# Kiteretsu77/This_and_That_VDM

Hardware: AMD Instinct MI355X
Metric: denoise-steps/sec (14-frame 256x448 VGL, 25 steps) (higher is better)
Workload: dtype bf16; 1 GPU; VGL denoise step: GestureNet ControlNet + spatio-temporal UNet + per-frame CFG + Euler, latent 14x4x32x56, CFG batch 2, 78 context tokens, heads (5,10,20,20); mode=vgl, requests_per_gpu=1, parallelism=1 independent request(s), one per GPU; RCCL weight broadcast at start-up only, hipgraph=True, finite_output=True, spatial_self_attention=bf16, weights_identical_on_all_ranks=True

## Files before the change

### this_and_that_vdm_amd/csrc/gemm.hip

```cpp
#include <stdlib.h>
#include "gemm_kernel.h"

namespace ttg {
void launch_bf16(GemmP& p, int cfg, hipStream_t st);
void launch_f16(GemmP& p, int cfg, hipStream_t st);
void launch_f32(GemmP& p, int cfg, hipStream_t st);
void launch_sq320_bf16(const GemmP& p, hipStream_t st);
void launch_sq320_f16(const GemmP& p, hipStream_t st);
void launch_pp_bf16(GemmP& p, hipStream_t st);
void launch_pp_f16(GemmP& p, hipStream_t st);
void launch_w320(GemmP& p, hipStream_t st, int bm, bool bf16);
}
using namespace ttg;

namespace {
inline int gemm_taps(int mode) { return mode == 1 || mode == 3 ? 9 : (mode == 2 ? 3 : 1); }

int env_int(const char* name, int dflt) { const char* e = getenv(name); return e ? atoi(e) : dflt; }
int big_tile_bits(int on) { return on == 0 ? 0 : (on == 2 ? 1 : (on == 3 ? 11 : (on == 4 ? 7 : 15))); }
struct Knobs {
  int forced_cfg = env_int("TT_GEMM_CFG", -1);
  int group_m = env_int("TT_GEMM_GROUP_M", 0);
  int forced_split = env_int("TT_GEMM_SPLITK", -1);
  int deep = env_int("TT_GEMM_DEEP", 1);
  int small64 = env_int("TT_GEMM_SMALL64", 2);
  int sq320 = env_int("TT_GEMM_SQ320", 2);
  int sq320_rowvec = env_int("TT_SQ320_ROWVEC", 1);
  int sq320_min_rows = env_int("TT_SQ320_MIN_ROWS", 131072);
  int pp = env_int("TT_GEMM_PP", 1);
  int pp_geglu_min_tiles = env_int("TT_PP_GEGLU_MIN_TILES", 400);
  int pp_geglu_min_fill = env_int("TT_PP_GEGLU_MIN_FILL", 75);
  int pp_min_tiles = env_int("TT_PP_MIN_TILES", 460);
  int pp_min_fill = env_int("TT_PP_MIN_FILL", 90);
  int pp_split_whole = env_int("TT_PP_SPLIT_WHOLE", 1);
  int w320 = big_tile_bits(env_int("TT_GEMM_W320", 1));
  int w320_force = env_int("TT_W320_FORCE", 0);
  int w320_min_fill = env_int("TT_W320_MIN_FILL", 60);
  int f32_split = env_int("TT_F32_SPLIT", 0) ? 1 : 0;
  int f32_split_min_tiles = env_int("TT_F32_SPLIT_MIN_TILES", 160);
  int f32_splitk = env_int("TT_F32_SPLITK", 1);
};
Knobs& knobs() { static Knobs k; return k; }

struct Plan { int cfg, splitk; };

Plan make_plan(int forced, int m, int n, long ktot, bool allow_split, bool wide_ok = true, bool mode0 = false, bool k128 = false) {
  Plan pl{0, 1};
  const int f = forced;
  const long b128 = (long)ceil_div(m, 128) * ceil_div(n, 128);
  const long b12864 = (long)ceil_div(m, 128) * ceil_div(n, 64);
  if (f >= 0 && f < kNumCfgs) pl.cfg = f;
  else if (n % 160 == 0 && n % 128 != 0 && n <= 960 && m >= 2048) pl.cfg = 7;
  else if (m >= 8192 && n >= 1024 && wide_ok) pl.cfg = 3;
  else if (m < 2048 && n >= 2560 && n % 160 == 0) pl.cfg = 7;
  else if (b128 >= 384) pl.cfg = 11;
  else if (b12864 >= 384) pl.cfg = 1;
  else pl.cfg = 2;
  const int fs = knobs().forced_split;
  if (fs >= 1) { pl.splitk = allow_split ? fs : 1; return pl; }
  const long kt = (ktot + 63) / 64;
  const int deep = knobs().deep;
  if (deep && f < 0 && b128 <= 256 && ktot > 0) {
    const int small64 = knobs().small64;
    if (small64 && (small64 != 2 || (m <= 64 && n >= 4096)) && mode0 && ktot <= 2048 && (long)ceil_div(m, 64) * ceil_div(n, 64) <= 512) { pl.cfg = 2; return pl; }
    pl.cfg = (deep == 2 && k128) ? 20 : 16;
    long s = allow_split ? 256 / b128 : 1;
    if (s > kt / 8) s = kt / 8;
    if (s > 16) s = 16;
    pl.splitk = s >= 2 ? (int)s : 1;
    return pl;
  }
  if (allow_split && f < 0 && b128 < 384 && kt >= 40) {
    long s = (512 + b128 - 1) / b128;
    if (s > kt / 8) s = kt / 8;
    if (s > 16) s = 16;
    if (s >= 2) { pl.cfg = 11; pl.splitk = (int)s; }
  }
  return pl;
}

int plan_f32(int m, int n, int min_tiles = 256) { return (long)ceil_div(m, 128) * ceil_div(n, 128) >= min_tiles ? 0 : 1; }

bool sq320_rowvec_ok(const TtGemmArgs* a) {
  if (!a->rowvec) return true;
  if (!knobs().sq320_rowvec || !a->residual) return false;
  if (a->rowvec_mod == 2 && a->rowvec_rows == 1) return true;
  return a->rowvec_mod == 0 && a->rowvec_rows >= 32 && a->rowvec_rows % 32 == 0 && (long)a->rowvec_rows * 2 >= a->m;
}
bool sq320_ok(const TtGemmArgs* a) {
  const int on = knobs().sq320;
  if (on == 2 && a->m < knobs().sq320_min_rows) return false;
  return on && a->dtype != TT_F32 && !a->ln_fold && !a->out_fp8 && knobs().forced_cfg < 0 && a->mode == 0 && a->k1 == 0 && a->k0 == SQ_K && a->n == SQ_N && a->m >= 4096 &&
         !a->geglu && sq320_rowvec_ok(a) && !a->out_f32 && !a->out_col_hw &&
         (!a->blend || (a->blend == a->residual && a->ld_blend == a->ld_res));
}
bool pp_ok(const TtGemmArgs* a) {
  const Knobs& k = knobs();
  if (!k.pp || k.forced_cfg >= 0 || a->dtype == TT_F32 || a->mode != 0 || a->k1 != 0 || a->ln_fold > 1 || a->out_fp8 || a->residual || a->blend ||
      a->rowvec || a->out_f32 || a->out_col_hw || (a->k0 & 63) || a->k0 < 128 || (a->n & 15) || (a->ldo & 7))
    return false;
  const long tiles = (long)ceil_div(a->m, 256) * ceil_div(a->n, 256);
  const long rounds = (tiles + 255) / 256;
  if (a->geglu) return tiles >= k.pp_geglu_min_tiles && tiles * 100 >= rounds * 256 * k.pp_geglu_min_fill;
  return tiles >= k.pp_min_tiles && tiles * 100 >= rounds * 256 * k.pp_min_fill;
}
bool w320_eligible(const TtGemmArgs* a) {
  if (!knobs().w320 || knobs().forced_cfg >= 0 || a->mode == 3 || a->dtype == TT_F32 || a->n % 320 || (a->k0 & 63) || (a->k1 & 63) || gemm_taps(a->mode) * (a->k0 + a->k1) < 128 || a->geglu ||
      a->out_fp8 || a->out_f32 || a->out_col_hw || a->ln_fold > 1 || (a->ln_fold && (a->mode != 0 || a->k1)))
    return false;
  if (a->mode == 1 && (a->stride != 1 || a->upsample || a->hin != a->hout || a->win != a->wout || a->win >= 32768 || a->hin >= 32768)) return false;
  if (a->rowvec && a->rowvec_rows < 32 && !(a->rowvec_rows == 1 && a->rowvec_mod == 2)) return false;
  if ((a->ldo & 3) || (a->residual && (a->ld_res & 3)) || (a->blend && (a->ld_blend & 3)) || (a->rowvec && (a->ld_rowvec & 3))) return false;
  if ((((size_t)a->out | (size_t)a->residual | (size_t)a->blend) & 7) || (((size_t)a->rowvec | (size_t)a->bias) & 15)) return false;
  return true;
}
int w320_route(const TtGemmArgs* a) {
  if (!w320_eligible(a)) return 0;
// ... 176 lines not shown
extern "C" int32_t tt_gemm_gn_fused(const TtGemmArgs* a) {
  if (!a || a->m <= 0 || a->n <= 0) return 0;
  return gn_fused_on(a, resolve(a));
}

extern "C" size_t tt_gemm_ws_bytes(const TtGemmArgs* a) {
  if (!a || a->m <= 0 || a->n <= 0) return 0;
  const Route r = wanted_route(a);
  if (r.kind == Kind::PP_TWO_PART) { TtGemmArgs head, tail; pp_split(a, r.head_rows, &head, &tail); return tt_gemm_ws_bytes(&tail); }
  return (r.kind == Kind::W320H_SPLIT || r.kind == Kind::TILED) && r.splitk > 1 ? slab_bytes(a, r.splitk) : 0;
}

namespace {
int fill_params(const TtGemmArgs* a, const Route& r, GemmP& p) {
  if (a->geglu && ((a->n & 15) || a->residual || a->blend || a->rowvec || a->out_f32 || a->out_col_hw))
    TT_FAIL(TT_EINVAL, "tt_gemm: geglu needs n %% 16 == 0 and no other epilogue terms");
  if (a->rowvec && a->rowvec_rows <= 0) TT_FAIL(TT_EINVAL, "tt_gemm: rowvec_rows");
  if (a->gn_out) {
    if (!a->gn_gamma || !a->gn_beta || (a->ld_gn & 3) || ((size_t)a->gn_out & 7)) TT_FAIL(TT_EINVAL, "tt_gemm: gn_out needs gn_gamma, gn_beta, ld_gn %% 4 == 0 and an 8-byte aligned pointer");
    if (!gn_fused_on(a, r)) TT_FAIL(TT_EUNSUPPORTED, "tt_gemm: gn_out on a problem without a split-K reduction pass (tt_gemm_gn_fused(args) == 0)");
  }
  if (a->stats_out && stats_rows_on(a, r) == 0)
    TT_FAIL(TT_EUNSUPPORTED, "tt_gemm: stats_out on a route without a statistics epilogue (tt_gemm_stats_rows(args) == 0)");
  if (a->rowvec_mod < 0 || (a->rowvec_mod > 0 && !a->rowvec)) TT_FAIL(TT_EINVAL, "tt_gemm: rowvec_mod %d (>= 0, needs rowvec)", a->rowvec_mod);
  if (a->ln_fold < 0 || a->ln_fold > 2) TT_FAIL(TT_EINVAL, "tt_gemm: ln_fold %d (0 none, 1 rows of A, 2 rows of W)", a->ln_fold);
  if (a->ln_fold && (a->mode != 0 || a->k1 != 0 || !(a->ln_eps > 0.f)))
    TT_FAIL(TT_EINVAL, "tt_gemm: ln_fold needs mode 0, one source spanning the whole LayerNorm row (k0 = C) and ln_eps > 0");
  if (a->ln_fold == 2 && a->geglu) TT_FAIL(TT_EINVAL, "tt_gemm: ln_fold 2 (columns) cannot be combined with geglu");
  if (a->out_fp8 && (a->dtype == TT_F32 || a->mode != 0 || a->geglu || a->residual || a->blend || a->rowvec || a->out_f32 || (a->ldo & 3)))
    TT_FAIL(TT_EINVAL, "tt_gemm: out_fp8 is for plain 16-bit linears (no geglu / residual / blend / rowvec / fp32 out), ldo %% 4 == 0");
  p.a0 = (const char*)a->a0; p.a1 = (const char*)a->a1; p.k0 = a->k0; p.k1 = a->k1;
  p.lda0 = a->lda0; p.lda1 = a->lda1; p.w = (const char*)a->w; p.ldw = a->ldw;
  p.m = a->m; p.n = a->n; p.mode = a->mode;
  p.nimg = a->nimg; p.hin = a->hin; p.win = a->win; p.hout = a->hout; p.wout = a->wout;
  p.stride = a->stride; p.upsample = a->upsample; p.frames = a->frames; p.hw = a->hw;
  p.bias = a->bias; p.acc_scale = a->acc_scale;
  p.rowvec = a->rowvec; p.rowvec_rows = a->rowvec_rows; p.ld_rowvec = a->ld_rowvec; p.rowvec_mod = a->rowvec ? a->rowvec_mod : 0;
  p.geglu = a->geglu; p.residual = (const char*)a->residual; p.ld_res = a->ld_res;
  p.blend = (const char*)a->blend; p.ld_blend = a->ld_blend; p.alpha = a->alpha;
  const int es = a->dtype == TT_F32 ? 4 : 2;
  p.out = (char*)a->out; p.ldo = a->ldo; p.out_f32 = a->dtype == TT_F32 ? 0 : a->out_f32;
  p.out_col_hw = a->out_col_hw; p.out_col_hwp = a->out_col_hwp;
  p.ln_fold = a->ln_fold; p.ln_eps = a->ln_eps; p.out_fp8 = a->out_fp8; p.stats = a->stats_out; p.stat_rows = a->gn_out ? a->stats_seg : (a->stats_out ? stats_rows_on(a, r) : 0);
  p.f32_split = a->dtype == TT_F32 ? knobs().f32_split : 0;
  p.presplit = a->presplit;
  if (a->presplit) {
    if ((a->presplit & ~3) || a->dtype != TT_F32 || !p.f32_split)
      TT_FAIL(TT_EINVAL, "tt_gemm: presplit operands need TT_F32 with tt_gemm_set_f32_split(1)");
    if (((a->presplit & 1) && a->ln_fold == 1) || ((a->presplit & 2) && a->ln_fold == 2))
      TT_FAIL(TT_EINVAL, "tt_gemm: the LayerNorm statistics cannot be taken from a pre-split operand");
    if ((a->presplit & 1) && a->mode != 0) TT_FAIL(TT_EINVAL, "tt_gemm: a pre-split A operand is a Linear operand (mode 0)");
  }
  p.gn_out = (char*)a->gn_out; p.ld_gn = a->ld_gn; p.gn_gamma = a->gn_gamma; p.gn_beta = a->gn_beta; p.gn_eps = a->gn_eps; p.gn_silu = a->gn_silu;
  if (p.mode == 1 || p.mode == 3) {
    if (p.nimg <= 0 || p.hin <= 0 || p.win <= 0 || p.hout <= 0 || p.wout <= 0 || p.stride < 1)
      TT_FAIL(TT_EINVAL, "tt_gemm: conv geometry");
    if ((long)p.nimg * p.hout * p.wout != p.m) TT_FAIL(TT_EINVAL, "tt_gemm: m != nimg*hout*wout");
  }
  if (p.mode == 2) {
    if (p.frames <= 0 || p.hw <= 0 || p.m % ((long)p.frames * p.hw)) TT_FAIL(TT_EINVAL, "tt_gemm: tconv geometry");
  }
  p.taps = gemm_taps(p.mode);
  {
    const long rows = p.mode == 1 || p.mode == 3 ? (long)p.nimg * p.hin * p.win : (long)p.m;
    const long a0b = ((rows - 1) * p.lda0 + p.k0) * es, a1b = p.k1 ? ((rows - 1) * p.lda1 + p.k1) * es : 16;
    const long wb = ((long)(p.n - 1) * p.ldw + (long)p.taps * (p.k0 + p.k1)) * es;
    if (a0b >= (1L << 31) || a1b >= (1L << 31) || wb >= (1L << 31))
      TT_FAIL(TT_EUNSUPPORTED, "tt_gemm: operand larger than 2 GiB (32-bit buffer offsets)");
    p.a0_bytes = (unsigned)a0b; p.a1_bytes = (unsigned)a1b; p.w_bytes = (unsigned)wb;
    const long n_out = p.geglu ? p.n / 2 : p.n;
    const long outb = ((long)(p.m - 1) * p.ldo + (p.out_col_hw > 0 ? p.ldo : n_out)) * (p.out_f32 ? 4 : (p.out_fp8 ? 1 : es));
    const long resb = p.residual ? ((long)(p.m - 1) * p.ld_res + p.n) * es : 0;
    const long blb = p.blend ? ((long)(p.m - 1) * p.ld_blend + p.n) * es : 0;
    long rv_last = p.rowvec ? (p.m - 1) / p.rowvec_rows : 0;
    if (p.rowvec_mod > 0 && rv_last > p.rowvec_mod - 1) rv_last = p.rowvec_mod - 1;
    const long rvb = p.rowvec ? (rv_last * p.ld_rowvec + p.n) * 4 : 0;
    if (outb >= (1L << 31) || resb >= (1L << 31) || blb >= (1L << 31) || rvb >= (1L << 31))
      TT_FAIL(TT_EUNSUPPORTED, "tt_gemm: epilogue operand larger than 2 GiB (32-bit buffer offsets)");
    p.out_bytes = (unsigned)outb; p.res_bytes = (unsigned)resb; p.blend_bytes = (unsigned)blb;
    p.bias_bytes = p.bias ? (unsigned)p.n * 4u : 0u; p.rowvec_bytes = (unsigned)rvb;
  }
  p.splitk = r.splitk; p.group_m = 1;
  p.group_m_override = r.kind == Kind::PP || r.kind == Kind::TILED ? knobs().group_m : 0;
  p.ws = r.splitk > 1 ? (float*)a->ws : nullptr;
  p.ws_bytes = r.splitk > 1 ? (unsigned)slab_bytes(a, r.splitk) : 0u;
  return TT_OK;
}
}

extern "C" int tt_gemm(const TtGemmArgs* a, tt_stream_t stream) {
  if (!a || !a->a0 || !a->w || !a->out) TT_FAIL(TT_EINVAL, "tt_gemm: null operand");
  if (a->m <= 0 || a->n <= 0 || a->k0 <= 0) TT_FAIL(TT_EINVAL, "tt_gemm: empty problem m=%d n=%d k0=%d", a->m, a->n, a->k0);
  if (a->dtype != TT_BF16 && a->dtype != TT_F16 && a->dtype != TT_F32) TT_FAIL(TT_EINVAL, "tt_gemm: bad dtype");
  if ((a->k0 & 7) || (a->k1 & 7) || (a->n & 3)) TT_FAIL(TT_EINVAL, "tt_gemm: k0/k1 must be multiples of 8 and n of 4");
  if ((a->lda0 & 7) || (a->k1 && (a->lda1 & 7)) || (a->ldw & 7)) TT_FAIL(TT_EINVAL, "tt_gemm: row strides must be multiples of 8 elements");
  if (a->k1 && !a->a1) TT_FAIL(TT_EINVAL, "tt_gemm: k1 > 0 without a1");
  if (a->mode < 0 || a->mode > 3) TT_FAIL(TT_EINVAL, "tt_gemm: bad mode %d", a->mode);
  if (a->mode == 3 && a->upsample) TT_FAIL(TT_EINVAL, "tt_gemm: mode 3 (bottom / right zero padding) has no fused upsample");
  const Route r = resolve(a);
  if (r.kind == Kind::PP_TWO_PART) {
    TtGemmArgs head, tail;
    pp_split(a, r.head_rows, &head, &tail);
    const int rc = tt_gemm(&head, stream);
    return rc != TT_OK ? rc : tt_gemm(&tail, stream);
  }
  GemmP p;
  if (const int rc = fill_params(a, r, p)) return rc;
  hipStream_t st = (hipStream_t)stream;
  const bool bf16 = a->dtype == TT_BF16;
  switch (r.kind) {
    case Kind::PP: if (bf16) launch_pp_bf16(p, st); else launch_pp_f16(p, st); break;
    case Kind::SQ320: if (bf16) launch_sq320_bf16(p, st); else launch_sq320_f16(p, st); break;
    case Kind::W320: launch_w320(p, st, 256, bf16); break;
    case Kind::W320H: case Kind::W320H_SPLIT: launch_w320(p, st, 128, bf16); break;
    case Kind::TILED:
      if (bf16) launch_bf16(p, r.cfg, st);
      else if (a->dtype == TT_F16) launch_f16(p, r.cfg, st);
      else launch_f32(p, r.cfg, st);
      break;
    default:
      TT_FAIL(TT_EUNSUPPORTED, "tt_gemm: forced tile configuration %d has no mode-3 variant (mode 3 is built for 1, 2, 11, 16)", r.cfg);
  }
  TT_CHECK_LAUNCH("tt_gemm");
  return TT_OK;
}
```

### this_and_that_vdm_amd/csrc/gemm_kernel.h

```cpp
#pragma once
#include <stdlib.h>
#include <type_traits>
#include "common.h"

namespace ttg {


struct FastDiv { unsigned mul, sh; };
static inline FastDiv make_fastdiv(long d_) {
  unsigned long long d = d_ < 1 ? 1 : (unsigned long long)d_;
  unsigned l = 0;
  while ((1ull << l) < d) ++l;
  FastDiv f;
  f.mul = (unsigned)(((1ull << (31 + l)) + d - 1) / d);
  f.sh = 31 + l;
  return f;
}
__device__ __forceinline__ int fdiv(int n, const FastDiv& f) { return (int)(((unsigned long long)(unsigned)n * f.mul) >> f.sh); }

struct GemmP {
  const char* a0; const char* a1;
  int k0, k1; long lda0, lda1;
  const char* w; long ldw;
  int m, n, mode;
  int nimg, hin, win, hout, wout, stride, upsample;
  int frames, hw;
  const float* bias; float acc_scale;
  const float* rowvec; int rowvec_rows; long ld_rowvec;
  int rowvec_mod;
  int geglu;
  const char* residual; long ld_res;
  const char* blend; long ld_blend; float alpha;
  char* out; long ldo; int out_f32;
  int out_col_hw, out_col_hwp;
  int nk0, nk1, taps, kt_total;
  int tiles_m, tiles_n;
  int group_m_override;
  int group_m;
  unsigned a0_bytes, a1_bytes, w_bytes;
  unsigned out_bytes, res_bytes, blend_bytes, bias_bytes, rowvec_bytes, ws_bytes;
  int splitk;
  float* ws;
  int ln_fold; float ln_eps;
  int out_fp8;
  float* stats;
  int stat_rows;
  char* gn_out; long ld_gn;
  const float* gn_gamma; const float* gn_beta; float gn_eps; int gn_silu;
  int f32_split;
  int presplit;
  FastDiv fd_splitk, fd_per_group, fd_group_m, fd_last_rows, fd_per_tap, fd_hwo, fd_wout, fd_hw, fd_frames, fd_rv_rows, fd_rv_mod;
};

__device__ __forceinline__ unsigned pack4_fp8(const float* v) {
  int w = 0;
  w = __builtin_amdgcn_cvt_pk_fp8_f32(__builtin_amdgcn_fmed3f(v[0], -448.f, 448.f), __builtin_amdgcn_fmed3f(v[1], -448.f, 448.f), w, false);
  w = __builtin_amdgcn_cvt_pk_fp8_f32(__builtin_amdgcn_fmed3f(v[2], -448.f, 448.f), __builtin_amdgcn_fmed3f(v[3], -448.f, 448.f), w, true);
  return (unsigned)w;
}
__device__ __forceinline__ void st32(__amdgpu_buffer_rsrc_t r, int off, unsigned a) {
  __builtin_amdgcn_raw_buffer_store_b32(a, r, off, 0, 0);
}

__device__ __forceinline__ void colstat_strip(const char* ebuf, int q_per_row, int lane, float* srow_sum, float* srow_sq, bool first) {
  if (lane < q_per_row * 4) {
    const int quad = lane >> 2, e4 = (lane & 3) * 4;
    float a = 0.f, b = 0.f;
#pragma unroll 8
    for (int r = 0; r < 32; ++r) {
      const float x = *(const float*)(ebuf + r * 256 + ((quad ^ (r & (q_per_row - 1))) << 4) + e4);
      a += x; b = fmaf(x, x, b);
    }
    if (!first) { a += srow_sum[lane]; b += srow_sq[lane]; }
    srow_sum[lane] = a; srow_sq[lane] = b;
  }
}

__device__ __forceinline__ void ln_stat_shifted(const raw_u32x4_t& f, float c, float& s, float& q) {
  const unsigned w[4] = {f.x, f.y, f.z, f.w};
#pragma unroll
  for (int d = 0; d < 4; ++d) { const float x = __uint_as_float(w[d]) - c; s += x; q = fmaf(x, x, q); }
}


#ifdef TT_GEMM_TIMELINE
static __device__ long long g_tl[8 * 8192];
#define TL(i) do { if (threadIdx.x == 0 && blockIdx.x < 8192) g_tl[blockIdx.x * 8 + (i)] = wall_clock64(); } while (0)
#else
#define TL(i) do { } while (0)
#endif

constexpr int kInv = (int)0x80000000;
typedef unsigned u32x2_t __attribute__((ext_vector_type(2)));
typedef unsigned u32x4_t __attribute__((ext_vector_type(4)));
__device__ __forceinline__ __amdgpu_buffer_rsrc_t make_rsrc(const void* ptr, unsigned bytes) {
  return __builtin_amdgcn_make_buffer_rsrc((void*)ptr, 0, (int)bytes, 0x00020000);
}
__device__ __forceinline__ uint2 ld64(__amdgpu_buffer_rsrc_t r, int off) {
  const u32x2_t v = __builtin_amdgcn_raw_buffer_load_b64(r, off, 0, 0);
  return make_uint2(v.x, v.y);
}
__device__ __forceinline__ float4 ld128f(__amdgpu_buffer_rsrc_t r, int off) {
  const u32x4_t v = __builtin_amdgcn_raw_buffer_load_b128(r, off, 0, 0);
  return make_float4(__uint_as_float(v.x), __uint_as_float(v.y), __uint_as_float(v.z), __uint_as_float(v.w));
}
__device__ __forceinline__ void st64(__amdgpu_buffer_rsrc_t r, int off, unsigned a, unsigned b) {
  __builtin_amdgcn_raw_buffer_store_b64((u32x2_t){a, b}, r, off, 0, 0);
}
__device__ __forceinline__ void st128f(__amdgpu_buffer_rsrc_t r, int off, float4 v) {
  __builtin_amdgcn_raw_buffer_store_b128((u32x4_t){__float_as_uint(v.x), __float_as_uint(v.y), __float_as_uint(v.z), __float_as_uint(v.w)}, r, off, 0, 0);
}
template <typename Tag> __device__ __forceinline__ typename Elem<Tag>::quad_t ldq(__amdgpu_buffer_rsrc_t r, int off) { return ld64(r, off); }
template <> __device__ __forceinline__ uint4 ldq<f32_tag>(__amdgpu_buffer_rsrc_t r, int off) {
  const u32x4_t v = __builtin_amdgcn_raw_buffer_load_b128(r, off, 0, 0);
  return make_uint4(v.x, v.y, v.z, v.w);
}
template <typename Tag> __device__ __forceinline__ void stq(__amdgpu_buffer_rsrc_t r, int off, const float* v) {
  st64(r, off, pack2<Tag>(v[0], v[1]), pack2<Tag>(v[2], v[3]));
}
template <> __device__ __forceinline__ void stq<f32_tag>(__amdgpu_buffer_rsrc_t r, int off, const float* v) {
  st128f(r, off, make_float4(v[0], v[1], v[2], v[3]));
// ... 1317 lines not shown
```

### this_and_that_vdm_amd/csrc/gemm_pp.hip

```cpp
#include <stdlib.h>
#include <type_traits>
#include "gemm_kernel.h"

#ifndef TT_PP_GEGLU_STORE_AUX
#define TT_PP_GEGLU_STORE_AUX 0
#endif

namespace ttg {

__device__ __forceinline__ void lds_write8_raw(unsigned addr, unsigned a, unsigned b) {
  const raw_u32x2_t v = {a, b};
  asm volatile("ds_write_b64 %0, %1" ::"v"(addr), "v"(v) : "memory");
}

template <typename Tag, int LNROWS, int GEGLU>
__global__ __launch_bounds__(512, 2) void gemm_pp_kernel(const GemmP p) {
  extern __shared__ __attribute__((aligned(16))) char smem[];
  kernarg_touch<sizeof(GemmP)>();
#ifdef TT_PP_HALF_PROBE
  constexpr int BM = 128, BN = 256, WTM = 64, WTN = 64, FM = 2, FN = 2, CPR = 8, ES = 2;
  constexpr bool HALF = true;
#else
  constexpr int BM = 256, BN = 256, WTM = 128, WTN = 64, FM = 4, FN = 2, CPR = 8, ES = 2;
  constexpr bool HALF = false;
#endif
  constexpr int REG = 16384, SLOT = 4 * REG, STRIP_OFF = 2 * SLOT;
  constexpr bool SPLIT = LNROWS && GEGLU;
  static_assert(Elem<Tag>::ES == 2, "16-bit storage types only");
  const int tid = threadIdx.x, lane = tid & 63;
  const int wid = __builtin_amdgcn_readfirstlane(tid >> 6);
  const int grp = wid >> 2, wr = wid >> 2, wc = wid & 3;
  const int l31 = lane & 31, hi = lane >> 5;
  const __amdgpu_buffer_rsrc_t ra = make_rsrc(p.a0, p.a0_bytes), rw = make_rsrc(p.w, p.w_bytes);
  const __amdgpu_buffer_rsrc_t rb = make_rsrc(p.bias, p.bias_bytes), ro = make_rsrc(p.out, p.out_bytes);
  const int KS = p.k0 >> 6;
  const int nwg = gridDim.x;
  const int ntiles = p.tiles_m * p.tiles_n;
  const int my_tiles = (int)blockIdx.x < ntiles ? (ntiles - 1 - (int)blockIdx.x) / nwg + 1 : 0;
  const int S = my_tiles * KS;
  auto tile_of = [&](int it, int& m0, int& n0) {
    const int bid = xcd_remap(it * nwg + (int)blockIdx.x, ntiles);
    const int gm = p.group_m, per_group = gm * p.tiles_n;
    const int g = bid / per_group, first = g * gm, rows = min(gm, p.tiles_m - first), rem = bid - g * per_group;
    const int tn = rem / rows, tm = first + (rem - tn * rows);
    m0 = tm * BM; n0 = tn * BN;
  };
  int pv[4][2];
  int p_it = 0, p_ks = 0;
  int q_m0[2] = {0, 0}, q_n0[2] = {0, 0};
  auto producer_tile = [&](int it) {
    int m0 = 0, n0 = 0;
    const bool ok = it < my_tiles;
    if (ok) tile_of(it, m0, n0);
    if (it & 1) { q_m0[1] = m0; q_n0[1] = n0; } else { q_m0[0] = m0; q_n0[0] = n0; }
#pragma unroll
    for (int i = 0; i < 2; ++i) {
      const int c = i * 512 + tid, rr = c >> 3, ch = (c & 7) ^ tile_swz<CPR>(rr);
      const int ar = HALF ? rr : (rr >> 6) * 128 + (rr & 63), br = (rr >> 5) * 64 + (rr & 31);
      pv[0][i] = (ok && m0 + ar < p.m) ? (int)(((long)(m0 + ar) * p.lda0 + ch * 8) * ES) : kInv;
      pv[1][i] = (!HALF && ok && m0 + ar + 64 < p.m) ? (int)(((long)(m0 + ar + 64) * p.lda0 + ch * 8) * ES) : kInv;
      pv[2][i] = (ok && n0 + br < p.n) ? (int)(((long)(n0 + br) * p.ldw + ch * 8) * ES) : kInv;
      pv[3][i] = (ok && n0 + br + 32 < p.n) ? (int)(((long)(n0 + br + 32) * p.ldw + ch * 8) * ES) : kInv;
    }
  };
  producer_tile(0);
  if (KS >= 5 && my_tiles > 0 && my_tiles * nwg < ntiles) {
    const int units = (int)blockIdx.x & 3;
    for (int u = 0; u < units; ++u) __builtin_amdgcn_s_sleep(127);
  }
  auto stage = [&](int slot, auto reg_tag) {
    constexpr int R = decltype(reg_tag)::value;
    char* base = smem + slot * SLOT + R * REG + wid * 1024;
    const int soff = __builtin_amdgcn_readfirstlane(p_ks) * 128;
#pragma unroll
    for (int i = 0; i < 2; ++i) {
      const int v = pv[R][i];
      if (R < 2) __builtin_amdgcn_raw_ptr_buffer_load_lds(ra, (__attribute__((address_space(3))) void*)(base + i * 8192), 16, v, soff, 0, 0);
      else __builtin_amdgcn_raw_ptr_buffer_load_lds(rw, (__attribute__((address_space(3))) void*)(base + i * 8192), 16, v, soff, 0, 0);
    }
    if constexpr (R == (HALF ? 3 : 2)) { if (++p_ks == KS) { p_ks = 0; ++p_it; producer_tile(p_it); } }
  };
  using R0 = std::integral_constant<int, 0>; using R1 = std::integral_constant<int, 1>;
  using R2 = std::integral_constant<int, 2>; using R3 = std::integral_constant<int, 3>;

  f32x16_t acc[FM][FN];
#pragma unroll
  for (int i = 0; i < FM; ++i)
#pragma unroll
    for (int j = 0; j < FN; ++j)
#pragma unroll
      for (int r = 0; r < 16; ++r) acc[i][j][r] = 0.f;
  float ln_s[FM], ln_q[FM];
#pragma unroll
  for (int i = 0; i < FM; ++i) ln_s[i] = ln_q[i] = 0.f;

  const unsigned lds_base = lds_addr(smem);
  unsigned a_addr[2][4], b_addr[4];
#pragma unroll
  for (int i = 0; i < 2; ++i) {
    const int rr = wr * 64 + i * 32 + l31;
#pragma unroll
    for (int ks = 0; ks < 4; ++ks) a_addr[i][ks] = rr * 128 + (((ks * 2 + hi) ^ tile_swz<CPR>(rr)) << 4);
  }
  {
    const int rr = wc * 32 + l31;
#pragma unroll
    for (int ks = 0; ks < 4; ++ks) b_addr[ks] = rr * 128 + (((ks * 2 + hi) ^ tile_swz<CPR>(rr)) << 4);
  }
  raw_u32x4_t af[2][4], bf[4];
  auto read_a = [&](unsigned sbase, int i2) {
#pragma unroll
    for (int i = 0; i < 2; ++i)
#pragma unroll
      for (int ks = 0; ks < 4; ++ks) af[i][ks] = lds_read16_raw(sbase + i2 * REG + a_addr[i][ks]);
  };
  auto read_b = [&](unsigned sbase, int j) {
#pragma unroll
    for (int ks = 0; ks < 4; ++ks) bf[ks] = lds_read16_raw(sbase + (2 + j) * REG + b_addr[ks]);
  };
  int c_ks = 0, c_it = 0;
  constexpr bool ZERO_BY_MFMA = GEGLU != 0;
  auto mma = [&](auto i2_tag, auto j_tag) {
    constexpr int I2 = decltype(i2_tag)::value, J = decltype(j_tag)::value;
    __builtin_amdgcn_s_setprio(1);
    if (ZERO_BY_MFMA && c_ks == 0) {
      f32x16_t z;
#pragma unroll
      for (int r = 0; r < 16; ++r) z[r] = 0.f;
#pragma unroll
      for (int ks = 0; ks < 4; ++ks)
#pragma unroll
        for (int i = 0; i < 2; ++i)
          acc[I2 * 2 + i][J] = Cvt<Tag>::mfma32(make_uint4(bf[ks].x, bf[ks].y, bf[ks].z, bf[ks].w),
                                                make_uint4(af[i][ks].x, af[i][ks].y, af[i][ks].z, af[i][ks].w), ks == 0 ? z : acc[I2 * 2 + i][J]);
    } else {
#pragma unroll
      for (int ks = 0; ks < 4; ++ks)
#pragma unroll
        for (int i = 0; i < 2; ++i)
          acc[I2 * 2 + i][J] = Cvt<Tag>::mfma32(make_uint4(bf[ks].x, bf[ks].y, bf[ks].z, bf[ks].w),
                                                make_uint4(af[i][ks].x, af[i][ks].y, af[i][ks].z, af[i][ks].w), acc[I2 * 2 + i][J]);
    }
    __builtin_amdgcn_s_setprio(0);
  };
  auto stats = [&](auto i2_tag) {
    constexpr int I2 = decltype(i2_tag)::value;
    if constexpr (LNROWS) {
#pragma unroll
      for (int ks = 0; ks < 4; ++ks)
        if (!SPLIT || ks == wc) {
#pragma unroll
          for (int i = 0; i < 2; ++i) ln_stat<Tag>(af[i][ks], ln_s[I2 * 2 + i], ln_q[I2 * 2 + i]);
        }
      __builtin_amdgcn_sched_barrier(0);
    }
  };
  auto bar = [&]() { __builtin_amdgcn_s_barrier(); asm volatile("" ::: "memory"); };
  using I0 = std::integral_constant<int, 0>; using I1 = std::integral_constant<int, 1>;

  if constexpr (HALF) {
    stage(0, R0{}); stage(0, R2{}); stage(0, R3{});
    stage(1, R0{}); stage(1, R2{});
    wait_vmcnt<4>();
  } else {
  stage(0, R0{}); stage(0, R3{}); stage(0, R1{}); stage(0, R2{});
  stage(1, R0{}); stage(1, R3{}); stage(1, R1{});
  wait_vmcnt<6>();
  }
  bar();
  if (grp == 1) bar();

  const unsigned strip = lds_base + STRIP_OFF + wid * 4096;

  int c_m0 = 0, c_n0 = 0;
  auto epilogue = [&]() {
    const int m0 = c_m0, n0 = c_n0;
    ++c_it;

    __builtin_amdgcn_sched_barrier(0);
    asm volatile("s_nop 15\n\ts_nop 15" ::: "memory");
    float4 b4[FN][4];
    {
      raw_u32x4_t t[FN][4];
#pragma unroll
      for (int j = 0; j < FN; ++j)
#pragma unroll
        for (int g = 0; g < 4; ++g) t[j][g] = lds_read16_raw(strip + (j * 32 + 8 * g + 4 * hi) * 4);
      lds_wait<0>();
#pragma unroll
      for (int j = 0; j < FN; ++j)
#pragma unroll
        for (int g = 0; g < 4; ++g)
          b4[j][g] = make_float4(__uint_as_float(t[j][g].x), __uint_as_float(t[j][g].y), __uint_as_float(t[j][g].z), __uint_as_float(t[j][g].w));
    }
    if constexpr (SPLIT) {
      lds_write16_raw(strip + 2048 + lane * 32, ln_s[0], ln_q[0], ln_s[1], ln_q[1]);
      if constexpr (FM == 4) lds_write16_raw(strip + 2048 + lane * 32 + 16, ln_s[FM - 2], ln_q[FM - 2], ln_s[FM - 1], ln_q[FM - 1]);
      lds_wait<0>();
      bar();
      raw_u32x4_t t[4][2];
      const unsigned row_strips = lds_base + STRIP_OFF + wr * 4 * 4096 + 2048 + lane * 32;
#pragma unroll
      for (int c = 0; c < 4; ++c) { t[c][0] = lds_read16_raw(row_strips + c * 4096); t[c][1] = lds_read16_raw(row_strips + c * 4096 + 16); }
      lds_wait<0>();
#pragma unroll
      for (int h = 0; h < FM / 2; ++h) {
        ln_s[2 * h] = (__uint_as_float(t[0][h].x) + __uint_as_float(t[1][h].x)) + (__uint_as_float(t[2][h].x) + __uint_as_float(t[3][h].x));
        ln_q[2 * h] = (__uint_as_float(t[0][h].y) + __uint_as_float(t[1][h].y)) + (__uint_as_float(t[2][h].y) + __uint_as_float(t[3][h].y));
        ln_s[2 * h + 1] = (__uint_as_float(t[0][h].z) + __uint_as_float(t[1][h].z)) + (__uint_as_float(t[2][h].z) + __uint_as_float(t[3][h].z));
        ln_q[2 * h + 1] = (__uint_as_float(t[0][h].w) + __uint_as_float(t[1][h].w)) + (__uint_as_float(t[2][h].w) + __uint_as_float(t[3][h].w));
      }
    }
    float rs[FM];
#pragma unroll
    for (int i = 0; i < FM; ++i) {
      rs[i] = 1.0f;
      if constexpr (LNROWS) {
        const float inv_k = 1.0f / (float)p.k0;
        const float sm = (ln_s[i] + __shfl_xor(ln_s[i], 32)) * inv_k, sq = (ln_q[i] + __shfl_xor(ln_q[i], 32)) * inv_k;
        rs[i] = rsqrtf(fmaxf(sq - sm * sm, 0.f) + p.ln_eps);
        ln_s[i] = ln_q[i] = 0.f;
      }
    }
    const float scale = p.acc_scale;
#pragma unroll
    for (int i = 0; i < FM; ++i) rs[i] *= scale;
#pragma unroll
    for (int j = 0; j < FN; ++j)
#pragma unroll
      for (int g = 0; g < 4; ++g) { b4[j][g].x *= scale; b4[j][g].y *= scale; b4[j][g].z *= scale; b4[j][g].w *= scale; }
#pragma unroll
    for (int i = 0; i < FM; ++i) {
      const int mb = m0 + wr * WTM + i * 32;
      if constexpr (!GEGLU) {
#pragma unroll
        for (int j = 0; j < FN; ++j)
#pragma unroll
          for (int g = 0; g < 4; ++g) {
            const float4 b = b4[j][g];
            const float v0 = fmaf(acc[i][j][g * 4], rs[i], b.x), v1 = fmaf(acc[i][j][g * 4 + 1], rs[i], b.y);
            const float v2 = fmaf(acc[i][j][g * 4 + 2], rs[i], b.z), v3 = fmaf(acc[i][j][g * 4 + 3], rs[i], b.w);
            const int col = j * 32 + 8 * g + 4 * hi;
            lds_write8_raw(strip + l31 * 128 + (((col >> 3) ^ (l31 & 7)) << 4) + ((col & 7) << 1), pack2<Tag>(v0, v1), pack2<Tag>(v2, v3));
          }
        raw_u32x4_t tq[4];
        const int ch = lane & 7, rr = lane >> 3;
#pragma unroll
        for (int ps = 0; ps < 4; ++ps) tq[ps] = lds_read16_raw(strip + (ps * 8 + rr) * 128 + ((ch ^ ((ps * 8 + rr) & 7)) << 4));
        lds_wait<0>();
        const int gn = n0 + wc * WTN + ch * 8;
#pragma unroll
        for (int ps = 0; ps < 4; ++ps) {
          const int gm = mb + ps * 8 + rr;
          __builtin_amdgcn_raw_buffer_store_b128((u32x4_t){tq[ps].x, tq[ps].y, tq[ps].z, tq[ps].w}, ro,
                                                 (gm < p.m && gn < p.n) ? (int)(((long)gm * p.ldo + gn) * ES) : kInv, 0, 0);
        }
      } else {
#pragma unroll
        for (int j = 0; j < FN; ++j)
#pragma unroll
          for (int tt = 0; tt < 2; ++tt) {
            const float4 bv = b4[j][2 * tt], bg = b4[j][2 * tt + 1];
            float v[4];
#ifdef TT_GELU_SCALAR
            const float bvv[4] = {bv.x, bv.y, bv.z, bv.w}, bgv[4] = {bg.x, bg.y, bg.z, bg.w};
#pragma unroll
            for (int e = 0; e < 4; ++e)
              v[e] = fmaf(acc[i][j][(2 * tt) * 4 + e], rs[i], bvv[e]) * gelu_erf_f(fmaf(acc[i][j][(2 * tt + 1) * 4 + e], rs[i], bgv[e]));
#else
            {
              const f32pk_t r2 = {rs[i], rs[i]};
              const f32pk_t g01 = (f32pk_t){acc[i][j][(2 * tt + 1) * 4], acc[i][j][(2 * tt + 1) * 4 + 1]} * r2 + (f32pk_t){bg.x, bg.y};
              const f32pk_t g23 = (f32pk_t){acc[i][j][(2 * tt + 1) * 4 + 2], acc[i][j][(2 * tt + 1) * 4 + 3]} * r2 + (f32pk_t){bg.z, bg.w};
#ifdef TT_GELU_ERF_AS
#define TT_PP_GELU gelu_erf_pk
#elif defined(TT_GELU_SIG)
#define TT_PP_GELU gelu_sig_pk
#else
#define TT_PP_GELU(x) (std::is_same<Tag, bf16_tag>::value ? gelu_poly_pk(x) : gelu_sig_pk(x))
#endif
              const f32pk_t v01 = ((f32pk_t){acc[i][j][(2 * tt) * 4], acc[i][j][(2 * tt) * 4 + 1]} * r2 + (f32pk_t){bv.x, bv.y}) * TT_PP_GELU(g01);
              const f32pk_t v23 = ((f32pk_t){acc[i][j][(2 * tt) * 4 + 2], acc[i][j][(2 * tt) * 4 + 3]} * r2 + (f32pk_t){bv.z, bv.w}) * TT_PP_GELU(g23);
              v[0] = v01.x; v[1] = v01.y; v[2] = v23.x; v[3] = v23.y;
            }
#endif
            const int col = j * 16 + tt * 8 + 4 * hi;
            lds_write8_raw(strip + l31 * 64 + (((col >> 3) ^ ((l31 >> 1) & 3)) << 4) + ((col & 7) << 1), pack2<Tag>(v[0], v[1]), pack2<Tag>(v[2], v[3]));
          }
        raw_u32x4_t tq[2];
        const int ch = lane & 3, rr = lane >> 2;
#pragma unroll
        for (int ps = 0; ps < 2; ++ps) tq[ps] = lds_read16_raw(strip + (ps * 16 + rr) * 64 + ((ch ^ (((ps * 16 + rr) >> 1) & 3)) << 4));
        lds_wait<0>();
        const int oc = ((n0 + wc * WTN) >> 1) + ch * 8;
#pragma unroll
        for (int ps = 0; ps < 2; ++ps) {
          const int gm = mb + ps * 16 + rr;
          __builtin_amdgcn_raw_buffer_store_b128((u32x4_t){tq[ps].x, tq[ps].y, tq[ps].z, tq[ps].w}, ro,
                                                 (gm < p.m && oc * 2 < p.n) ? (int)(((long)gm * p.ldo + oc) * ES) : kInv, 0, TT_PP_GEGLU_STORE_AUX);
        }
      }
      if constexpr (!ZERO_BY_MFMA) {
#pragma unroll
        for (int j = 0; j < FN; ++j)
#pragma unroll
          for (int r = 0; r < 16; ++r) acc[i][j][r] = 0.f;
      }
    }
  };

  for (int s = 0; s < S; ++s) {
    const int slot = s & 1;
    const unsigned sb = lds_base + slot * SLOT;
    if constexpr (HALF) {
      read_a(sb, 0); read_b(sb, 0);
      if (c_ks == 0) {
        const int m0 = (c_it & 1) ? q_m0[1] : q_m0[0], n0 = (c_it & 1) ? q_n0[1] : q_n0[0];
        c_m0 = m0; c_n0 = n0;
        const int gn = n0 + wc * 64 + lane;
        __builtin_amdgcn_raw_ptr_buffer_load_lds(rb, (__attribute__((address_space(3))) void*)(smem + STRIP_OFF + wid * 4096), 4,
                                                 gn < p.n ? gn * 4 : kInv, 0, 0, 0);
      }
      stage(slot ^ 1, R3{});
      lds_wait<0>();
      bar();
      mma(I0{}, I0{});
      bar();
      read_b(sb, 1);
      stage(slot, R0{}); stage(slot, R2{});
      stats(I0{});
      wait_vmcnt<4>();
      lds_wait<0>();
      bar();
      mma(I0{}, I1{});
      bar();
    } else {
    read_a(sb, 0); read_b(sb, 0);
    if (c_ks == 0) {
      const int m0 = (c_it & 1) ? q_m0[1] : q_m0[0], n0 = (c_it & 1) ? q_n0[1] : q_n0[0];
      c_m0 = m0; c_n0 = n0;
      const int gn = n0 + wc * 64 + lane;
      __builtin_amdgcn_raw_ptr_buffer_load_lds(rb, (__attribute__((address_space(3))) void*)(smem + STRIP_OFF + wid * 4096), 4,
                                               gn < p.n ? gn * 4 : kInv, 0, 0, 0);
    }
    stage(slot ^ 1, R2{});
    lds_wait<0>();
    bar();
    mma(I0{}, I0{});
    bar();
    read_b(sb, 1);
    stage(slot, R0{});
    stats(I0{});
    lds_wait<0>();
    bar();
    mma(I0{}, I1{});
    bar();
    read_a(sb, 1);
    stage(slot, R3{});
    lds_wait<0>();
    bar();
    mma(I1{}, I1{});
    bar();
    read_b(sb, 0);
    stage(slot, R1{});
    stats(I1{});
    wait_vmcnt<6>();
    lds_wait<0>();
    bar();
    mma(I1{}, I0{});
    bar();
    }
    if (++c_ks == KS) {
      c_ks = 0;
      if (grp == 0) bar();
      epilogue();
      if (grp == 1) bar();
    }
  }
}

template <typename Tag, int LNROWS, int GEGLU>
static void launch_pp_inst(GemmP& p, hipStream_t st) {
  constexpr int lds = 2 * 65536 + 8 * 4096;
  static unsigned long long attr_done = 0;
  tt_lds_opt_in((const void*)gemm_pp_kernel<Tag, LNROWS, GEGLU>, lds, &attr_done);
#ifdef TT_PP_HALF_PROBE
  p.tiles_m = ceil_div(p.m, 128);
#else
  p.tiles_m = ceil_div(p.m, 256);
#endif
  p.tiles_n = ceil_div(p.n, 256);
  int gm = 1;
  if (p.tiles_n > 8) while (gm * 2 * gm * 2 <= 32 && gm * 2 <= p.tiles_m) gm *= 2;
  p.group_m = p.group_m_override > 0 ? (p.group_m_override > p.tiles_m ? p.tiles_m : p.group_m_override) : gm;
  const int ntiles = p.tiles_m * p.tiles_n;
  hipLaunchKernelGGL((gemm_pp_kernel<Tag, LNROWS, GEGLU>), dim3(ntiles < 256 ? ntiles : 256), dim3(512), lds, st, p);
}
template <typename Tag>
static void launch_pp_tag(GemmP& p, hipStream_t st) {
  if (p.ln_fold) { if (p.geglu) launch_pp_inst<Tag, 1, 1>(p, st); else launch_pp_inst<Tag, 1, 0>(p, st); }
  else { if (p.geglu) launch_pp_inst<Tag, 0, 1>(p, st); else launch_pp_inst<Tag, 0, 0>(p, st); }
}
void launch_pp_bf16(GemmP& p, hipStream_t st) { launch_pp_tag<bf16_tag>(p, st); }
void launch_pp_f16(GemmP& p, hipStream_t st) { launch_pp_tag<f16_tag>(p, st); }

}
```

Baseline: 34.66 denoise-steps/s.

## Add contiguous tile walk to PP GEMM and reuse LayerNorm row stats across tiles

```diff
diff --git a/this_and_that_vdm_amd/csrc/gemm.hip b/this_and_that_vdm_amd/csrc/gemm.hip
--- a/this_and_that_vdm_amd/csrc/gemm.hip
+++ b/this_and_that_vdm_amd/csrc/gemm.hip
@@ -33,6 +33,7 @@
   int pp_min_tiles = env_int("TT_PP_MIN_TILES", 460);
   int pp_min_fill = env_int("TT_PP_MIN_FILL", 90);
   int pp_split_whole = env_int("TT_PP_SPLIT_WHOLE", 1);
+  int pp_walk = env_int("TT_PP_WALK", 0) ? 1 : 0;
   int w320 = big_tile_bits(env_int("TT_GEMM_W320", 1));
   int w320_force = env_int("TT_W320_FORCE", 0);
   int w320_min_fill = env_int("TT_W320_MIN_FILL", 60);
@@ -375,6 +376,7 @@
   }
   p.splitk = r.splitk; p.group_m = 1;
   p.group_m_override = r.kind == Kind::PP || r.kind == Kind::TILED ? knobs().group_m : 0;
+  p.walk = knobs().pp_walk;
   p.ws = r.splitk > 1 ? (float*)a->ws : nullptr;
   p.ws_bytes = r.splitk > 1 ? (unsigned)slab_bytes(a, r.splitk) : 0u;
   return TT_OK;
diff --git a/this_and_that_vdm_amd/csrc/gemm_kernel.h b/this_and_that_vdm_amd/csrc/gemm_kernel.h
--- a/this_and_that_vdm_amd/csrc/gemm_kernel.h
+++ b/this_and_that_vdm_amd/csrc/gemm_kernel.h
@@ -37,6 +37,7 @@
   int tiles_m, tiles_n;
   int group_m_override;
   int group_m;
+  int walk;
   unsigned a0_bytes, a1_bytes, w_bytes;
   unsigned out_bytes, res_bytes, blend_bytes, bias_bytes, rowvec_bytes, ws_bytes;
   int splitk;
diff --git a/this_and_that_vdm_amd/csrc/gemm_pp.hip b/this_and_that_vdm_amd/csrc/gemm_pp.hip
--- a/this_and_that_vdm_amd/csrc/gemm_pp.hip
+++ b/this_and_that_vdm_amd/csrc/gemm_pp.hip
@@ -36,9 +36,17 @@
   const int KS = p.k0 >> 6;
   const int nwg = gridDim.x;
   const int ntiles = p.tiles_m * p.tiles_n;
-  const int my_tiles = (int)blockIdx.x < ntiles ? (ntiles - 1 - (int)blockIdx.x) / nwg + 1 : 0;
-  const int S = my_tiles * KS;
+  const int wj = (nwg & 7) ? (int)blockIdx.x : ((int)blockIdx.x & 7) * (nwg >> 3) + ((int)blockIdx.x >> 3);
+  const int t_first = (int)((long)wj * ntiles / nwg);
+  const int my_tiles = p.walk ? (int)((long)(wj + 1) * ntiles / nwg) - t_first
+                              : ((int)blockIdx.x < ntiles ? (ntiles - 1 - (int)blockIdx.x) / nwg + 1 : 0);
+  int w_m0 = t_first / p.tiles_n * BM, w_n0 = t_first % p.tiles_n * BN;
   auto tile_of = [&](int it, int& m0, int& n0) {
+    if (p.walk) {
+      if (it > 0) { w_n0 += BN; if (w_n0 >= p.n) { w_n0 = 0; w_m0 += BM; } }
+      m0 = w_m0; n0 = w_n0;
+      return;
+    }
     const int bid = xcd_remap(it * nwg + (int)blockIdx.x, ntiles);
     const int gm = p.group_m, per_group = gm * p.tiles_n;
     const int g = bid / per_group, first = g * gm, rows = min(gm, p.tiles_m - first), rem = bid - g * per_group;
@@ -47,15 +55,17 @@
   };
   int pv[4][2];
   int p_it = 0, p_ks = 0;
-  int q_m0[2] = {0, 0}, q_n0[2] = {0, 0};
+  int q_m0a = 0, q_m0b = 0, q_n0a = 0, q_n0b = 0;
   auto producer_tile = [&](int it) {
     int m0 = 0, n0 = 0;
     const bool ok = it < my_tiles;
     if (ok) tile_of(it, m0, n0);
-    if (it & 1) { q_m0[1] = m0; q_n0[1] = n0; } else { q_m0[0] = m0; q_n0[0] = n0; }
+    if (it & 1) { q_m0b = m0; q_n0b = n0; } else { q_m0a = m0; q_n0a = n0; }
+    int t = tid;
+    asm volatile("" : "+v"(t));
 #pragma unroll
     for (int i = 0; i < 2; ++i) {
-      const int c = i * 512 + tid, rr = c >> 3, ch = (c & 7) ^ tile_swz<CPR>(rr);
+      const int c = i * 512 + t, rr = c >> 3, ch = (c & 7) ^ tile_swz<CPR>(rr);
       const int ar = HALF ? rr : (rr >> 6) * 128 + (rr & 63), br = (rr >> 5) * 64 + (rr & 31);
       pv[0][i] = (ok && m0 + ar < p.m) ? (int)(((long)(m0 + ar) * p.lda0 + ch * 8) * ES) : kInv;
       pv[1][i] = (!HALF && ok && m0 + ar + 64 < p.m) ? (int)(((long)(m0 + ar + 64) * p.lda0 + ch * 8) * ES) : kInv;
@@ -91,8 +101,9 @@
 #pragma unroll
       for (int r = 0; r < 16; ++r) acc[i][j][r] = 0.f;
   float ln_s[FM], ln_q[FM];
-#pragma unroll
-  for (int i = 0; i < FM; ++i) ln_s[i] = ln_q[i] = 0.f;
+  float ln_rs[FM];
+#pragma unroll
+  for (int i = 0; i < FM; ++i) { ln_s[i] = ln_q[i] = 0.f; ln_rs[i] = 1.0f; }
 
   const unsigned lds_base = lds_addr(smem);
   unsigned a_addr[2][4], b_addr[4];
@@ -118,12 +129,11 @@
 #pragma unroll
     for (int ks = 0; ks < 4; ++ks) bf[ks] = lds_read16_raw(sbase + (2 + j) * REG + b_addr[ks]);
   };
-  int c_ks = 0, c_it = 0;
   constexpr bool ZERO_BY_MFMA = GEGLU != 0;
-  auto mma = [&](auto i2_tag, auto j_tag) {
+  auto mma = [&](auto i2_tag, auto j_tag, auto first_tag) {
     constexpr int I2 = decltype(i2_tag)::value, J = decltype(j_tag)::value;
     __builtin_amdgcn_s_setprio(1);
-    if (ZERO_BY_MFMA && c_ks == 0) {
+    if constexpr (ZERO_BY_MFMA && decltype(first_tag)::value) {
       f32x16_t z;
 #pragma unroll
       for (int r = 0; r < 16; ++r) z[r] = 0.f;
@@ -143,9 +153,9 @@
     }
     __builtin_amdgcn_s_setprio(0);
   };
-  auto stats = [&](auto i2_tag) {
+  auto stats = [&](auto i2_tag, auto sum_tag) {
     constexpr int I2 = decltype(i2_tag)::value;
-    if constexpr (LNROWS) {
+    if constexpr (LNROWS && decltype(sum_tag)::value) {
 #pragma unroll
       for (int ks = 0; ks < 4; ++ks)
         if (!SPLIT || ks == wc) {
@@ -170,12 +180,15 @@
   bar();
   if (grp == 1) bar();
 
-  const unsigned strip = lds_base + STRIP_OFF + wid * 4096;
+  const unsigned strip_k = lds_base + STRIP_OFF + wid * 4096;
 
   int c_m0 = 0, c_n0 = 0;
   auto epilogue = [&]() {
     const int m0 = c_m0, n0 = c_n0;
-    ++c_it;
+    unsigned strip = strip_k; int lane = tid;
+    asm volatile("" : "+v"(strip), "+v"(lane));
+    lane &= 63;
+    const int l31 = lane & 31, hi = lane >> 5;
 
     __builtin_amdgcn_sched_barrier(0);
     asm volatile("s_nop 15\n\ts_nop 15" ::: "memory");
@@ -193,35 +206,9 @@
         for (int g = 0; g < 4; ++g)
           b4[j][g] = make_float4(__uint_as_float(t[j][g].x), __uint_as_float(t[j][g].y), __uint_as_float(t[j][g].z), __uint_as_float(t[j][g].w));
     }
-    if constexpr (SPLIT) {
-      lds_write16_raw(strip + 2048 + lane * 32, ln_s[0], ln_q[0], ln_s[1], ln_q[1]);
-      if constexpr (FM == 4) lds_write16_raw(strip + 2048 + lane * 32 + 16, ln_s[FM - 2], ln_q[FM - 2], ln_s[FM - 1], ln_q[FM - 1]);
-      lds_wait<0>();
-      bar();
-      raw_u32x4_t t[4][2];
-      const unsigned row_strips = lds_base + STRIP_OFF + wr * 4 * 4096 + 2048 + lane * 32;
-#pragma unroll
-      for (int c = 0; c < 4; ++c) { t[c][0] = lds_read16_raw(row_strips + c * 4096); t[c][1] = lds_read16_raw(row_strips + c * 4096 + 16); }
-      lds_wait<0>();
-#pragma unroll
-      for (int h = 0; h < FM / 2; ++h) {
-        ln_s[2 * h] = (__uint_as_float(t[0][h].x) + __uint_as_float(t[1][h].x)) + (__uint_as_float(t[2][h].x) + __uint_as_float(t[3][h].x));
-        ln_q[2 * h] = (__uint_as_float(t[0][h].y) + __uint_as_float(t[1][h].y)) + (__uint_as_float(t[2][h].y) + __uint_as_float(t[3][h].y));
-        ln_s[2 * h + 1] = (__uint_as_float(t[0][h].z) + __uint_as_float(t[1][h].z)) + (__uint_as_float(t[2][h].z) + __uint_as_float(t[3][h].z));
-        ln_q[2 * h + 1] = (__uint_as_float(t[0][h].w) + __uint_as_float(t[1][h].w)) + (__uint_as_float(t[2][h].w) + __uint_as_float(t[3][h].w));
-      }
-    }
     float rs[FM];
 #pragma unroll
-    for (int i = 0; i < FM; ++i) {
-      rs[i] = 1.0f;
-      if constexpr (LNROWS) {
-        const float inv_k = 1.0f / (float)p.k0;
-        const float sm = (ln_s[i] + __shfl_xor(ln_s[i], 32)) * inv_k, sq = (ln_q[i] + __shfl_xor(ln_q[i], 32)) * inv_k;
-        rs[i] = rsqrtf(fmaxf(sq - sm * sm, 0.f) + p.ln_eps);
-        ln_s[i] = ln_q[i] = 0.f;
-      }
-    }
+    for (int i = 0; i < FM; ++i) rs[i] = LNROWS ? ln_rs[i] : 1.0f;
     const float scale = p.acc_scale;
 #pragma unroll
     for (int i = 0; i < FM; ++i) rs[i] *= scale;
@@ -309,13 +296,47 @@
     }
   };
 
-  for (int s = 0; s < S; ++s) {
+  auto finish_stats = [&]() {
+    __builtin_amdgcn_sched_barrier(0);
+    unsigned strip = strip_k; int lane = tid, ks64 = KS;
+    asm volatile("" : "+v"(strip), "+v"(lane), "+s"(ks64));
+    lane &= 63;
+    const float inv_k = 1.0f / (float)(ks64 << 6);
+    const int other = (lane ^ 32) << 2;
+    auto swap32 = [&](float v) { return __int_as_float(__builtin_amdgcn_ds_bpermute(other, __float_as_int(v))); };
+    if constexpr (SPLIT) {
+      lds_write16_raw(strip + 2048 + lane * 32, ln_s[0], ln_q[0], ln_s[1], ln_q[1]);
+      if constexpr (FM == 4) lds_write16_raw(strip + 2048 + lane * 32 + 16, ln_s[FM - 2], ln_q[FM - 2], ln_s[FM - 1], ln_q[FM - 1]);
+      lds_wait<0>();
+      bar();
+      raw_u32x4_t t[4][2];
+      const unsigned row_strips = lds_base + STRIP_OFF + wr * 4 * 4096 + 2048 + lane * 32;
+#pragma unroll
+      for (int c = 0; c < 4; ++c) { t[c][0] = lds_read16_raw(row_strips + c * 4096); t[c][1] = lds_read16_raw(row_strips + c * 4096 + 16); }
+      lds_wait<0>();
+#pragma unroll
+      for (int h = 0; h < FM / 2; ++h) {
+        ln_s[2 * h] = (__uint_as_float(t[0][h].x) + __uint_as_float(t[1][h].x)) + (__uint_as_float(t[2][h].x) + __uint_as_float(t[3][h].x));
+        ln_q[2 * h] = (__uint_as_float(t[0][h].y) + __uint_as_float(t[1][h].y)) + (__uint_as_float(t[2][h].y) + __uint_as_float(t[3][h].y));
+        ln_s[2 * h + 1] = (__uint_as_float(t[0][h].z) + __uint_as_float(t[1][h].z)) + (__uint_as_float(t[2][h].z) + __uint_as_float(t[3][h].z));
+        ln_q[2 * h + 1] = (__uint_as_float(t[0][h].w) + __uint_as_float(t[1][h].w)) + (__uint_as_float(t[2][h].w) + __uint_as_float(t[3][h].w));
+      }
+    }
+#pragma unroll
+    for (int i = 0; i < FM; ++i) {
+      const float sm = (ln_s[i] + swap32(ln_s[i])) * inv_k, sq = (ln_q[i] + swap32(ln_q[i])) * inv_k;
+      ln_rs[i] = rsqrtf(fmaxf(sq - sm * sm, 0.f) + p.ln_eps);
+    }
+  };
+
+  int s = 0;
+  auto slab = [&](int it, auto sum_tag, auto first_tag) {
     const int slot = s & 1;
     const unsigned sb = lds_base + slot * SLOT;
     if constexpr (HALF) {
       read_a(sb, 0); read_b(sb, 0);
-      if (c_ks == 0) {
-        const int m0 = (c_it & 1) ? q_m0[1] : q_m0[0], n0 = (c_it & 1) ? q_n0[1] : q_n0[0];
+      if constexpr (decltype(first_tag)::value) {
+        const int m0 = (it & 1) ? q_m0b : q_m0a, n0 = (it & 1) ? q_n0b : q_n0a;
         c_m0 = m0; c_n0 = n0;
         const int gn = n0 + wc * 64 + lane;
         __builtin_amdgcn_raw_ptr_buffer_load_lds(rb, (__attribute__((address_space(3))) void*)(smem + STRIP_OFF + wid * 4096), 4,
@@ -324,20 +345,20 @@
       stage(slot ^ 1, R3{});
       lds_wait<0>();
       bar();
-      mma(I0{}, I0{});
+      mma(I0{}, I0{}, first_tag);
       bar();
       read_b(sb, 1);
       stage(slot, R0{}); stage(slot, R2{});
-      stats(I0{});
+      stats(I0{}, sum_tag);
       wait_vmcnt<4>();
       lds_wait<0>();
       bar();
-      mma(I0{}, I1{});
+      mma(I0{}, I1{}, first_tag);
       bar();
     } else {
     read_a(sb, 0); read_b(sb, 0);
-    if (c_ks == 0) {
-      const int m0 = (c_it & 1) ? q_m0[1] : q_m0[0], n0 = (c_it & 1) ? q_n0[1] : q_n0[0];
+    if constexpr (decltype(first_tag)::value) {
+      const int m0 = (it & 1) ? q_m0b : q_m0a, n0 = (it & 1) ? q_n0b : q_n0a;
       c_m0 = m0; c_n0 = n0;
       const int gn = n0 + wc * 64 + lane;
       __builtin_amdgcn_raw_ptr_buffer_load_lds(rb, (__attribute__((address_space(3))) void*)(smem + STRIP_OFF + wid * 4096), 4,
@@ -346,36 +367,53 @@
     stage(slot ^ 1, R2{});
     lds_wait<0>();
     bar();
-    mma(I0{}, I0{});
+    mma(I0{}, I0{}, first_tag);
     bar();
     read_b(sb, 1);
     stage(slot, R0{});
-    stats(I0{});
+    stats(I0{}, sum_tag);
     lds_wait<0>();
     bar();
-    mma(I0{}, I1{});
+    mma(I0{}, I1{}, first_tag);
     bar();
     read_a(sb, 1);
     stage(slot, R3{});
     lds_wait<0>();
     bar();
-    mma(I1{}, I1{});
+    mma(I1{}, I1{}, first_tag);
     bar();
     read_b(sb, 0);
     stage(slot, R1{});
-    stats(I1{});
+    stats(I1{}, sum_tag);
     wait_vmcnt<6>();
     lds_wait<0>();
     bar();
-    mma(I1{}, I0{});
-    bar();
-    }
-    if (++c_ks == KS) {
-      c_ks = 0;
+    mma(I1{}, I0{}, first_tag);
+    bar();
+    }
+    ++s;
+  };
+  using SumYes = std::integral_constant<bool, true>; using SumNo = std::integral_constant<bool, false>;
+  using First = std::integral_constant<bool, true>; using Later = std::integral_constant<bool, false>;
+  for (int it = 0; it < my_tiles; ++it) {
+    bool reuse = false;
+    if constexpr (LNROWS) reuse = __builtin_amdgcn_readfirstlane(p.walk && it > 0 && ((it & 1) ? q_m0b : q_m0a) == c_m0);
+    if (reuse) {
+      slab(it, SumNo{}, First{});
+      for (int ks = 1; ks < KS; ++ks) slab(it, SumNo{}, Later{});
       if (grp == 0) bar();
-      epilogue();
-      if (grp == 1) bar();
-    }
+    } else {
+      if constexpr (LNROWS) {
+#pragma unroll
+        for (int i = 0; i < FM; ++i) ln_s[i] = ln_q[i] = 0.f;
+      }
+      slab(it, SumYes{}, First{});
+      for (int ks = 1; ks < KS; ++ks) slab(it, SumYes{}, Later{});
+      if (grp == 0) bar();
+      if constexpr (LNROWS) finish_stats();
+    }
+    epilogue();
+    if (grp == 1) bar();
   }
 }
 
```

Result: no change. 34.69 denoise-steps/s, median of 3 (+0.1%).
